# netease-youdao/EmotiVoice

Measured on NVIDIA H100. Metric: mel_frames_per_sec, higher is better.
Workload: dtype fp32 (fp32 storage + accumulate; tensor-core fp32 emulation: 3xTF32 prefix, bf16x3 after it)

## Files before the change

### emotivoice_b200/build.py

```python
import hashlib
import os
import subprocess
import sys

HERE = os.path.dirname(os.path.abspath(__file__))
CSRC = os.path.join(HERE, "csrc")
LIB_DIR = os.path.join(HERE, "lib")
LIB_PATH = os.path.join(LIB_DIR, "libemotivoice_b200.so")
INCLUDE = os.path.join(os.path.dirname(HERE), "include")

NVCC_FLAGS = ["-gencode", "arch=compute_90a,code=sm_90a", "-lineinfo", "-O3", "-std=c++17",
              "-Xcompiler", "-fPIC,-fvisibility=hidden", "-cudart", "static"]


def sources():
    return sorted(os.path.join(CSRC, f) for f in os.listdir(CSRC) if f.endswith(".cu"))


def _digest():
    h = hashlib.sha256()
    files = sources() + sorted(os.path.join(CSRC, f) for f in os.listdir(CSRC) if f.endswith(".cuh"))
    files.append(os.path.join(INCLUDE, "emotivoice_b200.h"))
    for f in files:
        h.update(os.path.basename(f).encode())
        with open(f, "rb") as fh:
            h.update(fh.read())
    h.update(" ".join(NVCC_FLAGS).encode())
    return h.hexdigest()


def nvcc_path():
    for c in (os.environ.get("NVCC"), "/usr/local/cuda/bin/nvcc", "nvcc"):
        if c and (os.path.isabs(c) and os.path.exists(c) or not os.path.isabs(c)):
            return c
    return "nvcc"


def build(force=False, verbose=True):
    import fcntl
    if not force and _up_to_date(_digest()):
        if verbose:
            print("emotivoice_b200.build: up to date, not recompiled", flush=True)
        return LIB_PATH
    os.makedirs(LIB_DIR, exist_ok=True)
    with open(os.path.join(LIB_DIR, ".build.lock"), "w") as lock:
        fcntl.flock(lock, fcntl.LOCK_EX)
        try:
            return _build_locked(force, verbose)
        finally:
            fcntl.flock(lock, fcntl.LOCK_UN)


def _up_to_date(dig):
    stamp = os.path.join(LIB_DIR, "build.stamp")
    if not (os.path.exists(LIB_PATH) and os.path.exists(stamp)):
        return False
    with open(stamp) as f:
        return f.read().strip() == dig


def _build_locked(force, verbose):
    stamp = os.path.join(LIB_DIR, "build.stamp")
    dig = _digest()
    if not force and _up_to_date(dig):
        if verbose:
            print("emotivoice_b200.build: up to date (sources digest %s), not recompiled" % dig[:12], flush=True)
        return LIB_PATH
    objs = []
    procs = []
    for src in sources():
        obj = os.path.join(LIB_DIR, os.path.basename(src)[:-3] + ".o")
        objs.append(obj)
        cmd = [nvcc_path()] + NVCC_FLAGS + ["-I", INCLUDE, "-c", src, "-o", obj]
        if verbose:
            print(" ".join(cmd), flush=True)
        procs.append((src, subprocess.Popen(cmd, stdout=subprocess.PIPE, stderr=subprocess.STDOUT)))
    serialised = []
    for src, p in procs:
        out, _ = p.communicate()
        if p.returncode != 0:
            sys.stderr.write(out.decode())
            raise RuntimeError("nvcc failed on %s" % src)
        if verbose and out.strip():
            print(out.decode())
        if b"C7520" in out:
            if not verbose:
                sys.stderr.write(out.decode())
            serialised.append(os.path.basename(src))
    if serialised:
        raise RuntimeError("ptxas serialised wgmma instructions (warning C7520, reason above) in %s; a wgmma on a path ptxas cannot "
                           "prove warp-uniform is one cause" % ", ".join(serialised))
    cmd = [nvcc_path(), "-shared", "-o", LIB_PATH] + objs + ["-cudart", "static",
                                                           "-gencode", "arch=compute_90a,code=sm_90a"]
    if verbose:
        print(" ".join(cmd), flush=True)
    subprocess.check_call(cmd)
    with open(stamp, "w") as f:
        f.write(dig)
    if verbose:
        print("emotivoice_b200.build: compiled %d sources with nvcc for sm_90a (digest %s)" % (len(objs), dig[:12]), flush=True)
    return LIB_PATH


if __name__ == "__main__":
    print(build(force="--force" in sys.argv))
```

### emotivoice_b200/csrc/conv1d_tc.cu

```cuda
#include <cstdio>
#include <cstdlib>

#include "ev_common.cuh"
#include "tc_common.cuh"

namespace ev {

namespace tc {

struct Plan {
  int BN, mt, kbg, planes;
  int rows_pad;
  int a_plane_bytes, b_plane_bytes, a_stage_bytes, b_stage_bytes;
  int a_stages, b_stages;
  int ngroups;
  int ksplit;
  int acc_cols;
  int tiles_m, tiles_n, total_tiles;
  int smem_total;
};

__host__ __device__ inline bool make_plan(const ConvParams& p, int mode, int BN, int mt, int kbg, int min_b_stages, Plan* o, int b_target = 4) {
  Plan q;
  q.planes = (mode == 1 || mode == 3) ? 2 : 1;
  const int cpg = mode >= 2 ? 8 : 4;
  q.kbg = kbg;
  q.mt = mt;
  q.BN = BN;
  if (mt * q.BN > 2 * ACC_REGS) return false;
  q.acc_cols = mt * q.BN;
  const int rows = BM * mt + (p.K - 1) * p.dil;
  q.rows_pad = ((rows + 7) / 8) * 8 + 8 / q.kbg;
  q.a_plane_bytes = q.kbg * q.rows_pad * 16;
  q.b_plane_bytes = q.kbg * q.BN * 16;
  q.a_stage_bytes = q.planes * q.a_plane_bytes;
  q.b_stage_bytes = q.planes * q.b_plane_bytes;
  const int budget = 227 * 1024 - 1024;
  const int n_cb = (p.Cin + cpg * q.kbg - 1) / (cpg * q.kbg);
  if (min_b_stages > n_cb * p.K) min_b_stages = n_cb * p.K;
  if (min_b_stages < 2) min_b_stages = 2;
  if (2 * q.a_stage_bytes + min_b_stages * q.b_stage_bytes > budget) return false;
  q.a_stages = 2;
  q.b_stages = 2;
  while (q.b_stages < MAX_B_STAGES && q.b_stages < n_cb * p.K &&
         q.a_stages * q.a_stage_bytes + (q.b_stages + 1) * q.b_stage_bytes <= budget && q.b_stages < b_target) ++q.b_stages;
  while (q.a_stages < MAX_A_STAGES && q.a_stages < n_cb &&
         (q.a_stages + 1) * q.a_stage_bytes + q.b_stages * q.b_stage_bytes <= budget && q.a_stages < 6) ++q.a_stages;
  while (q.b_stages < MAX_B_STAGES && q.b_stages < n_cb * p.K &&
         q.a_stages * q.a_stage_bytes + (q.b_stages + 1) * q.b_stage_bytes <= budget) ++q.b_stages;
  while (q.a_stages < MAX_A_STAGES && q.a_stages < n_cb &&
         (q.a_stages + 1) * q.a_stage_bytes + q.b_stages * q.b_stage_bytes <= budget) ++q.a_stages;
  q.ngroups = q.a_stages >= 6 ? 6 : (q.a_stages >= 3 ? 3 : (q.a_stages >= 2 ? 2 : 1));
  q.tiles_m = (p.L + BM * mt - 1) / (BM * mt);
  q.tiles_n = (p.Cout + q.BN - 1) / q.BN;
  q.ksplit = 1;
  q.total_tiles = p.B * q.tiles_m * q.tiles_n;
  q.smem_total = 1024 + q.a_stages * q.a_stage_bytes + q.b_stages * q.b_stage_bytes;
  *o = q;
  return true;
}

__device__ __forceinline__ void splitk_reduce_store(const ConvParams& p, int S, size_t per, size_t e, int b, int row, int col, int len) {
  float4 o = make_float4(0.f, 0.f, 0.f, 0.f);
  if (row < len) {
    for (int z = 0; z < S; ++z) {
      const float4 v = *reinterpret_cast<const float4*>(p.splitk_ws + (size_t)z * per + e);
      o.x += v.x; o.y += v.y; o.z += v.z; o.w += v.w;
    }
    if (p.bias) {
      const float4 b4 = __ldg(reinterpret_cast<const float4*>(p.bias + (size_t)b * p.bias_bs + col));
      o.x += b4.x; o.y += b4.y; o.z += b4.z; o.w += b4.w;
    }
    if (p.out_act != EV_ACT_NONE) {
      o.x = act_apply(o.x, p.out_act, 0.f); o.y = act_apply(o.y, p.out_act, 0.f);
      o.z = act_apply(o.z, p.out_act, 0.f); o.w = act_apply(o.w, p.out_act, 0.f);
    }
    if (p.res) {
      const float4 r4 = *reinterpret_cast<const float4*>(p.res + e);
      o.x += r4.x; o.y += r4.y; o.z += r4.z; o.w += r4.w;
    }
    if (p.acc != EV_ACC_STORE) {
      const float4 q4 = *reinterpret_cast<const float4*>(p.out + e);
      o.x += q4.x; o.y += q4.y; o.z += q4.z; o.w += q4.w;
      if (p.acc == EV_ACC_ADD_DIV) { o.x /= p.div; o.y /= p.div; o.z /= p.div; o.w /= p.div; }
    }
  }
  *reinterpret_cast<float4*>(p.out + e) = o;
}

template <int MODE, int MT, int KBG, int BN>
__global__ void __launch_bounds__(NTHREADS, 1) conv1d_tc_kernel(ConvParams p, Plan pl) {
  constexpr bool SPLIT3 = (MODE == 1);
  constexpr bool X3B = (MODE == 3);
  constexpr bool BF16 = (MODE == 2) || X3B;
  constexpr int PLANES = (SPLIT3 || X3B) ? 2 : 1;
  constexpr int CPG = BF16 ? 8 : 4;
  constexpr int KB = CPG * KBG;
  constexpr int NK8 = KBG / 2;
  constexpr int GSH = (KBG == 8 ? 3 : 2);
  constexpr int NA = BN / 2;
  constexpr int NCW = NCONS / 32;
  static_assert(BN % 16 == 0 && MT * BN <= 2 * ACC_REGS, "accumulators of the tile exceed the register budget");
  extern __shared__ __align__(128) uint8_t smem_raw[];
  const int tid = threadIdx.x;
  const int warp = __shfl_sync(0xffffffffu, tid >> 5, 0);
  const int lane = tid & 31;

  uint64_t* bars = reinterpret_cast<uint64_t*>(smem_raw);
  uint8_t* a_tiles = smem_raw + 1024;
  uint8_t* b_tiles = a_tiles + pl.a_stages * pl.a_stage_bytes;
  const uint32_t bar_base = smem_u32(bars);
  auto a_full = [&](int s) { return bar_base + 8u * s; };
  auto a_empty = [&](int s) { return bar_base + 8u * (MAX_A_STAGES + s); };
  auto b_full = [&](int s) { return bar_base + 8u * (2 * MAX_A_STAGES + s); };
  auto b_empty = [&](int s) { return bar_base + 8u * (2 * MAX_A_STAGES + MAX_B_STAGES + s); };

  if (tid == 0) {
    for (int s = 0; s < pl.a_stages; ++s) { mbar_init(a_full(s), (NPWARPS / pl.ngroups) * 32); mbar_init(a_empty(s), NCW); }
    for (int s = 0; s < pl.b_stages; ++s) { mbar_init(b_full(s), 1); mbar_init(b_empty(s), NCW); }
    asm volatile("fence.mbarrier_init.release.cluster;" ::: "memory");
  }
  __syncthreads();

  asm volatile("griddepcontrol.launch_dependents;" ::: "memory");

  const int n_cb = (p.Cin + KB - 1) / KB;
  const int halo = ((p.K - 1) / 2) * p.dil;
  const int rows_a = BM * MT + (p.K - 1) * p.dil;
  const int tiles_per_b = pl.tiles_m * pl.tiles_n;

  int z_cur = 0;
  auto decode = [&](int tile, int& b, int& t0, int& n0, int& nt, int& len) {
    z_cur = tile % pl.ksplit;
    tile /= pl.ksplit;
    b = tile / tiles_per_b;
    const int r = tile - b * tiles_per_b;
    const int tm = r / pl.tiles_n, tn = r - tm * pl.tiles_n;
    t0 = tm * (BM * MT);
    n0 = tn * BN;
    nt = min(BN, p.Cout - n0);
    len = p.lens ? min(p.L, p.lens[b] * p.lens_mul) : p.L;
  };

  if (warp < NCW) {
    asm volatile("griddepcontrol.wait;" ::: "memory");
    const int wg = warp >> 2, wl = warp & 3;
    const bool split = pl.ksplit > 1;
    const bool has_res = p.res != nullptr && !split;
    const int oact = split ? EV_ACT_NONE : p.out_act, accm = split ? EV_ACC_STORE : p.acc;
    const uint32_t a_lbo = (uint32_t)pl.rows_pad * 16u, b_lbo = (uint32_t)BN * 16u;
    const uint64_t a_desc0 = make_desc(0u, a_lbo, 128u), b_desc0 = make_desc(0u, b_lbo, 128u);
    const uint32_t a_tap = (uint32_t)p.dil * 16u, a_k8 = 2u * a_lbo;
    float acc[MT][NA];
#pragma unroll
    for (int mt = 0; mt < MT; ++mt)
#pragma unroll
      for (int i = 0; i < NA; ++i) acc[mt][i] = 0.f;
    auto release = [&](int sb, int sa) {
      __syncwarp();
      if (lane == 0) {
        mbar_arrive(b_empty(sb));
        if (sa >= 0) mbar_arrive(a_empty(sa));
      }
    };
    int a_cnt = 0, b_cnt = 0;
    for (int tile = blockIdx.x; tile < pl.total_tiles; tile += gridDim.x) {
      int b, t0, n0, nt, len;
      decode(tile, b, t0, n0, nt, len);
      float* ob = (split ? p.splitk_ws + (size_t)z_cur * p.B * p.L * p.Cout : p.out) + (size_t)b * p.L * p.Cout;
      const float* rb = has_res ? p.res + (size_t)b * p.L * p.Cout : nullptr;
      const bool active = t0 < len;
      if (active) {
        const int cb_lo = (z_cur * n_cb) / pl.ksplit, cb_hi = ((z_cur + 1) * n_cb) / pl.ksplit;
        int prev_sb = -1, prev_sa = -1;
        for (int cb = cb_lo; cb < cb_hi; ++cb, ++a_cnt) {
          const int sa = a_cnt % pl.a_stages;
          const int nk8 = min(KB, p.Cin - cb * KB) / (2 * CPG);
          mbar_wait(a_full(sa), (a_cnt / pl.a_stages) & 1);
          const uint64_t a_hi0 = desc_advance(a_desc0, smem_u32(a_tiles + sa * pl.a_stage_bytes) + (uint32_t)(wg * 64) * 16u);
          for (int j = 0; j < p.K; ++j, ++b_cnt) {
            const int sb = b_cnt % pl.b_stages;
            mbar_wait(b_full(sb), (b_cnt / pl.b_stages) & 1);
            const uint64_t b_hi0 = desc_advance(b_desc0, smem_u32(b_tiles + sb * pl.b_stage_bytes));
            const uint64_t a_j = desc_advance(a_hi0, (uint32_t)j * a_tap);
            if (nk8 == NK8) {
              tap_chain<MODE, BN, NK8>(acc, a_j, a_k8, (uint32_t)pl.a_plane_bytes, b_hi0, (uint32_t)pl.b_plane_bytes, (cb - cb_lo) | j);
              wgmma_wait<1>();
            } else {
              tap_chain_short<MODE, BN>(acc, a_j, a_k8, (uint32_t)pl.a_plane_bytes, b_hi0, (uint32_t)pl.b_plane_bytes, (cb - cb_lo) | j, nk8);
              wgmma_wait<1>();
            }
            if (prev_sb >= 0) release(prev_sb, prev_sa);
            prev_sb = sb;
            prev_sa = j == p.K - 1 ? sa : -1;
          }
        }
        wgmma_wait<0>();
        release(prev_sb, prev_sa);
      }
      const float* __restrict__ bias = (p.bias && !split) ? p.bias + (size_t)b * p.bias_bs + n0 : nullptr;
#pragma unroll
      for (int mt = 0; mt < MT; ++mt) {
#pragma unroll
        for (int i = 0; i < NA; i += 2) {
          const int c = frag_col(i, lane);
          const int row = t0 + mt * BM + wg * 64 + frag_row(i, lane, wl);
          if (c >= nt || row >= p.L) continue;
          const size_t off = (size_t)row * p.Cout + n0 + c;
          float2 o = make_float2(0.f, 0.f);
          if (active && row < len) {
            o = make_float2(acc[mt][i], acc[mt][i + 1]);
            if (bias) {
              const float2 b2 = __ldg(reinterpret_cast<const float2*>(bias + c));
              o.x += b2.x; o.y += b2.y;
            }
            if (oact != EV_ACT_NONE) { o.x = act_apply(o.x, oact, 0.f); o.y = act_apply(o.y, oact, 0.f); }
            if (has_res) {
              const float2 r2 = *reinterpret_cast<const float2*>(rb + off);
              o.x += r2.x; o.y += r2.y;
            }
            if (accm != EV_ACC_STORE) {
              const float2 q2 = *reinterpret_cast<const float2*>(ob + off);
              o.x += q2.x; o.y += q2.y;
              if (accm == EV_ACC_ADD_DIV) { o.x /= p.div; o.y /= p.div; }
            }
          }
          *reinterpret_cast<float2*>(ob + off) = o;
        }
      }
    }
  } else if (warp < W_WLOAD) {
    asm volatile("griddepcontrol.wait;" ::: "memory");
    const int pwarp = warp - NCW;
    const int wpg = NPWARPS / pl.ngroups;
    const int grp = pwarp / wpg;
    const int gt = (pwarp - grp * wpg) * 32 + lane;
    const int GT = wpg * 32;
    const bool lrelu = (p.in_act == EV_ACT_LRELU);
    const float slope = p.in_slope;
    const int total = rows_a * KBG;
    int a_cnt = 0;
    for (int tile = blockIdx.x; tile < pl.total_tiles; tile += gridDim.x) {
      int b, t0, n0, nt, len;
      decode(tile, b, t0, n0, nt, len);
      if (t0 >= len) continue;
      const float* __restrict__ xb = p.x + (size_t)b * p.L * p.Cin;
      const int cb_lo = (z_cur * n_cb) / pl.ksplit, cb_hi = ((z_cur + 1) * n_cb) / pl.ksplit;
      for (int cb = cb_lo; cb < cb_hi; ++cb, ++a_cnt) {
        if (a_cnt % pl.ngroups != grp) continue;
        const int s = a_cnt % pl.a_stages;
        const int c0 = cb * KB;
        const int ngran = min(KB, p.Cin - c0) / CPG;
        uint8_t* dst = a_tiles + s * pl.a_stage_bytes;
        constexpr int ALD = BF16 ? A_LD / 2 : A_LD;
        constexpr int NW = BF16 ? 2 : 1;
        for (int base = 0; base < total; base += GT * ALD) {
          float4 v[ALD * NW];
#pragma unroll
          for (int u = 0; u < ALD; ++u) {
            const int idx = base + u * GT + gt;
            const int r = idx >> GSH, g = idx & (KBG - 1);
            const int row = t0 - halo + r;
            const bool ok = idx < total && g < ngran && row >= 0 && row < len;
            const float* src = xb + (size_t)row * p.Cin + c0 + g * CPG;
#pragma unroll
            for (int w = 0; w < NW; ++w)
              v[u * NW + w] = ok ? __ldg(reinterpret_cast<const float4*>(src + 4 * w)) : make_float4(0.f, 0.f, 0.f, 0.f);
          }
          if (base == 0) mbar_wait(a_empty(s), ((a_cnt / pl.a_stages) & 1) ^ 1);
#pragma unroll
          for (int u = 0; u < ALD; ++u) {
            const int idx = base + u * GT + gt;
            const int r = idx >> GSH, g = idx & (KBG - 1);
            if (idx < total && g < ngran) {
#pragma unroll
              for (int w = 0; w < NW; ++w) {
                float4& t = v[u * NW + w];
                if (lrelu) {
                  t.x = t.x > 0.f ? t.x : t.x * slope;
                  t.y = t.y > 0.f ? t.y : t.y * slope;
                  t.z = t.z > 0.f ? t.z : t.z * slope;
                  t.w = t.w > 0.f ? t.w : t.w * slope;
                }
              }
              uint8_t* d = dst + ((size_t)g * pl.rows_pad + r) * 16;
              if (BF16) {
                const float4 t0 = v[u * NW], t1 = v[u * NW + NW - 1];
                uint4 q;
                q.x = pack_bf16(t0.x, t0.y); q.y = pack_bf16(t0.z, t0.w);
                q.z = pack_bf16(t1.x, t1.y); q.w = pack_bf16(t1.z, t1.w);
                *reinterpret_cast<uint4*>(d) = q;
                if (X3B) {
                  uint4 l;
                  l.x = pack_bf16(t0.x - __uint_as_float(q.x << 16), t0.y - __uint_as_float(q.x & 0xffff0000u));
                  l.y = pack_bf16(t0.z - __uint_as_float(q.y << 16), t0.w - __uint_as_float(q.y & 0xffff0000u));
                  l.z = pack_bf16(t1.x - __uint_as_float(q.z << 16), t1.y - __uint_as_float(q.z & 0xffff0000u));
                  l.w = pack_bf16(t1.z - __uint_as_float(q.w << 16), t1.w - __uint_as_float(q.w & 0xffff0000u));
                  *reinterpret_cast<uint4*>(d + pl.a_plane_bytes) = l;
                }
              } else {
                const float4 t = v[u * NW];
                const float4 h = make_float4(to_tf32(t.x), to_tf32(t.y), to_tf32(t.z), to_tf32(t.w));
                *reinterpret_cast<float4*>(d) = h;
                if (SPLIT3) {
                  const float4 l = make_float4(to_tf32(t.x - h.x), to_tf32(t.y - h.y), to_tf32(t.z - h.z), to_tf32(t.w - h.w));
                  *reinterpret_cast<float4*>(d + pl.a_plane_bytes) = l;
                }
              }
            }
          }
        }
        fence_proxy_async();
        mbar_arrive(a_full(s));
      }
    }
  } else {
    if (lane == 0) {
      asm volatile("griddepcontrol.wait;" ::: "memory");
      const int cin4 = p.Cin / CPG;
      const int bnp = p.Cout < 128 ? p.Cout : 128;
      const size_t plane = (size_t)p.K * cin4 * p.Cout * 4;
      const size_t tile_stride = (size_t)p.K * cin4 * bnp * 4;
      int b_cnt = 0;
      for (int tile = blockIdx.x; tile < pl.total_tiles; tile += gridDim.x) {
        int b, t0, n0, nt, len;
        decode(tile, b, t0, n0, nt, len);
        if (t0 >= len) continue;
        const float* wt = p.w + (size_t)(n0 / bnp) * tile_stride + (size_t)(n0 % bnp) * 4;
        const int cb_lo = (z_cur * n_cb) / pl.ksplit, cb_hi = ((z_cur + 1) * n_cb) / pl.ksplit;
        for (int cb = cb_lo; cb < cb_hi; ++cb) {
          const int ngran = min(KB, p.Cin - cb * KB) / CPG;
          for (int j = 0; j < p.K; ++j, ++b_cnt) {
            const int sb = b_cnt % pl.b_stages;
            mbar_wait(b_empty(sb), ((b_cnt / pl.b_stages) & 1) ^ 1);
            mbar_expect_tx(b_full(sb), (uint32_t)(PLANES * ngran * nt * 16));
            const uint32_t dst = smem_u32(b_tiles + sb * pl.b_stage_bytes);
            const float* src = wt + ((size_t)j * cin4 + (size_t)cb * KBG) * bnp * 4;
            if (nt == bnp) {
              bulk_g2s(dst, src, (uint32_t)(ngran * nt * 16), b_full(sb));
              if (PLANES == 2) bulk_g2s(dst + (uint32_t)pl.b_plane_bytes, src + plane, (uint32_t)(ngran * nt * 16), b_full(sb));
            } else {
              for (int g = 0; g < ngran; ++g) {
                bulk_g2s(dst + (uint32_t)(g * BN * 16), src + (size_t)g * bnp * 4, (uint32_t)(nt * 16), b_full(sb));
                if (PLANES == 2) bulk_g2s(dst + (uint32_t)(pl.b_plane_bytes + g * BN * 16), src + plane + (size_t)g * bnp * 4, (uint32_t)(nt * 16), b_full(sb));
              }
            }
          }
        }
      }
    }
    __syncwarp();
  }
}

__global__ void __launch_bounds__(256) splitk_reduce_kernel(ConvParams p, int S) {
  pdl_entry();
  const size_t per = (size_t)p.B * p.L * p.Cout;
  const size_t i4 = (size_t)blockIdx.x * blockDim.x + threadIdx.x;
  if (i4 * 4 >= per) return;
  const size_t e = i4 * 4;
  const int col = (int)(e % p.Cout);
  const size_t rowg = e / p.Cout;
  const int b = (int)(rowg / p.L), row = (int)(rowg % p.L);
  const int len = p.lens ? min(p.L, p.lens[b] * p.lens_mul) : p.L;
  splitk_reduce_store(p, S, per, e, b, row, col, len);
}

}

using TcKernel = void (*)(ConvParams, tc::Plan);
template <int MODE, int KBG>
static TcKernel tc_kernel_tile(int mt, int bn) {
  using namespace tc;
  switch (bn) {
    case 128: return mt == 1 ? conv1d_tc_kernel<MODE, 1, KBG, 128> : nullptr;
    case 112: return mt == 1 ? conv1d_tc_kernel<MODE, 1, KBG, 112> : nullptr;
    case 96: return mt == 1 ? conv1d_tc_kernel<MODE, 1, KBG, 96> : nullptr;
    case 80: return mt == 1 ? conv1d_tc_kernel<MODE, 1, KBG, 80> : nullptr;
    case 64: return mt == 2 ? conv1d_tc_kernel<MODE, 2, KBG, 64> : mt == 1 ? conv1d_tc_kernel<MODE, 1, KBG, 64> : nullptr;
    case 48: return mt == 2 ? conv1d_tc_kernel<MODE, 2, KBG, 48> : mt == 1 ? conv1d_tc_kernel<MODE, 1, KBG, 48> : nullptr;
    case 32: return mt == 4 ? conv1d_tc_kernel<MODE, 4, KBG, 32> : mt == 2 ? conv1d_tc_kernel<MODE, 2, KBG, 32>
                  : mt == 1 ? conv1d_tc_kernel<MODE, 1, KBG, 32> : nullptr;
    case 16: return mt == 4 ? conv1d_tc_kernel<MODE, 4, KBG, 16> : mt == 2 ? conv1d_tc_kernel<MODE, 2, KBG, 16>
                  : mt == 1 ? conv1d_tc_kernel<MODE, 1, KBG, 16> : nullptr;
    default: return nullptr;
  }
}
static TcKernel tc_kernel(int mode, int kbg, int mt, int bn) {
  if (mode == 1) return kbg == 4 ? tc_kernel_tile<1, 4>(mt, bn) : nullptr;
  if (mode == 3) return kbg == 8 ? tc_kernel_tile<3, 8>(mt, bn) : tc_kernel_tile<3, 4>(mt, bn);
  if (mode == 2) return kbg == 8 ? tc_kernel_tile<2, 8>(mt, bn) : tc_kernel_tile<2, 4>(mt, bn);
  return kbg == 8 ? tc_kernel_tile<0, 8>(mt, bn) : tc_kernel_tile<0, 4>(mt, bn);
}

void preload_conv1d_tc() {
  for (int mode = 0; mode < 4; ++mode)
    for (int kbg = 4; kbg <= 8; kbg += 4)
      for (int bn = 16; bn <= 128; bn += 16)
        for (int mt = 1; mt <= 4 && mt * bn <= 128; mt *= 2)
          if (const TcKernel k = tc_kernel(mode, kbg, mt, bn)) cudaFuncSetAttribute(k, cudaFuncAttributeMaxDynamicSharedMemorySize, 227 * 1024);
  cudaFuncAttributes fa;
  cudaFuncGetAttributes(&fa, tc::splitk_reduce_kernel);
  cudaGetLastError();
}

static int validate_conv1d_tc(const ConvParams& p, int mode) {
  EV_CHECK_ARG(p.B > 0 && p.L > 0, "conv1d_tc: bad problem B=%d L=%d", p.B, p.L);
  EV_CHECK_ARG(p.Cin % (mode >= 2 ? 16 : 8) == 0, "conv1d_tc: Cin=%d must be a multiple of %d", p.Cin, mode >= 2 ? 16 : 8);
  EV_CHECK_ARG(p.Cout % 16 == 0 && (p.Cout <= 128 || p.Cout % 128 == 0), "conv1d_tc: Cout=%d must be a multiple of 16, and of 128 above 128", p.Cout);
  EV_CHECK_ARG(p.K >= 1 && (p.K & 1) && p.dil >= 1, "conv1d_tc: K=%d must be odd, dil=%d >= 1", p.K, p.dil);
  EV_CHECK_ARG(p.in_act == EV_ACT_NONE || p.in_act == EV_ACT_LRELU, "conv1d_tc: unsupported input activation");
  return EV_OK;
}

int tc_shape_kbg(const ConvParams& p, int mode) {
  tc::Plan pl;
  const int bn_max = p.Cout <= 128 ? p.Cout : 128;
  return (mode != 1 && tc::make_plan(p, mode, bn_max, 1, 8, 4, &pl)) ? 8 : 4;
}

static int apply_ksplit(const ConvParams& p, int mode, tc::Plan* pl) {
  const size_t per = (size_t)p.B * p.L * p.Cout;
  if (p.ksplit > 1 && (p.splitk_ws || p.splitk_cap == (size_t)-1)) {
    int S = p.ksplit;
    const int cpg = mode >= 2 ? 8 : 4;
    const int n_cb = (p.Cin + cpg * pl->kbg - 1) / (cpg * pl->kbg);
    if (S > n_cb) S = n_cb;
    if ((size_t)S * per > p.splitk_cap) { set_error("conv1d_tc: split-K scratch too small (%zu < %zu floats)", p.splitk_cap, (size_t)S * per); return EV_EWORKSPACE; }
    if (S > 1) {
      pl->ksplit = S;
      pl->total_tiles *= S;
    }
  }
  return EV_OK;
}

static int plan_conv1d_tc(const ConvParams& p, int mode, tc::Plan* out) {
  EV_TRY(validate_conv1d_tc(p, mode));
  const int bn_thresh = 24, mt_thresh = 120;
  const long long tiles128 = (long long)((p.L + tc::BM - 1) / tc::BM) * p.B;
  int BN = p.Cout <= 128 ? p.Cout : 128;
  while (BN >= 64 && (BN / 2) % 16 == 0 && tiles128 * ((p.Cout + BN - 1) / BN) < bn_thresh) BN /= 2;
  int mt = tiles128 >= 4 * mt_thresh ? 4 : (tiles128 >= 2 * mt_thresh ? 2 : 1);
  tc::Plan pl;
  const int kbg = tc_shape_kbg(p, mode);
  for (;; mt >>= 1) {
    if (tc::make_plan(p, mode, BN, mt, kbg, 4, &pl)) break;
    if (tc::make_plan(p, mode, BN, mt, kbg, 2, &pl)) break;
    if (mt == 1) { set_error("conv1d_tc: tile does not fit in shared memory / accumulator registers (K=%d dil=%d Cout=%d)", p.K, p.dil, p.Cout); return EV_EINVAL; }
  }
  EV_TRY(apply_ksplit(p, mode, &pl));
  *out = pl;
  return EV_OK;
}

int debug_tc_plan(const ConvParams& p, int mode, int* v) {
  tc::Plan pl;
  const int rc = plan_conv1d_tc(p, mode, &pl);
  if (rc != EV_OK) return rc;
  v[0] = pl.BN; v[1] = pl.mt; v[2] = pl.kbg; v[3] = pl.a_stages; v[4] = pl.b_stages; v[5] = pl.ngroups;
  v[6] = pl.ksplit; v[7] = pl.acc_cols; v[8] = pl.smem_total; v[9] = pl.total_tiles; v[10] = pl.rows_pad;
  return EV_OK;
}

static int dispatch_tc(const ConvParams& p, int mode, const tc::Plan& pl, cudaStream_t st) {
  static std::atomic<uint64_t> attr_devs{0};
  if (first_use_on_device(attr_devs)) preload_conv1d_tc();
  const TcKernel k = tc_kernel(mode, pl.kbg, pl.mt, pl.BN);
  EV_CHECK_ARG(k, "conv1d_tc: no kernel for mode %d, KBG %d, MT %d, BN %d", mode, pl.kbg, pl.mt, pl.BN);
  const int grid = pl.total_tiles < sm_count() ? pl.total_tiles : sm_count();
  return launch("conv1d_tc_kernel", k, (unsigned)grid, tc::NTHREADS, pl.smem_total, st, p, pl);
}

int launch_conv1d_tc(const ConvParams& p, int mode, cudaStream_t st) {
  tc::Plan pl;
  EV_TRY(plan_conv1d_tc(p, mode, &pl));
  const size_t per = (size_t)p.B * p.L * p.Cout;
  const int rc = dispatch_tc(p, mode, pl, st);
  if (rc != EV_OK || pl.ksplit == 1) return rc;
  const size_t n4 = per / 4;
  return launch("splitk_reduce_kernel", tc::splitk_reduce_kernel, (unsigned)((n4 + 255) / 256), 256, 0, st, p, pl.ksplit);
}

}
```

Before: 126,500.

## Prefetch first weight stages before PDL grid-dependency wait in conv kernel

The weight-loader warp now issues bulk copies for the first block's initial B stages before griddepcontrol.wait, because the weights do not depend on the previous kernel. This overlaps weight fetch with the tail of the preceding launch. The consumer drains those early stages when the first tile is skipped. The change also adds an optional globaltimer timeline instrumentation build, compiled out by default.

```diff
diff --git a/emotivoice_b200/build.py b/emotivoice_b200/build.py
--- a/emotivoice_b200/build.py
+++ b/emotivoice_b200/build.py
@@ -66,12 +66,21 @@
         if verbose:
             print("emotivoice_b200.build: up to date (sources digest %s), not recompiled" % dig[:12], flush=True)
         return LIB_PATH
+    _compile(LIB_PATH, LIB_DIR, NVCC_FLAGS, verbose)
+    with open(stamp, "w") as f:
+        f.write(dig)
+    if verbose:
+        print("emotivoice_b200.build: compiled %d sources with nvcc for sm_90a (digest %s)" % (len(sources()), dig[:12]), flush=True)
+    return LIB_PATH
+
+
+def _compile(lib_path, obj_dir, flags, verbose):
     objs = []
     procs = []
     for src in sources():
-        obj = os.path.join(LIB_DIR, os.path.basename(src)[:-3] + ".o")
+        obj = os.path.join(obj_dir, os.path.basename(src)[:-3] + ".o")
         objs.append(obj)
-        cmd = [nvcc_path()] + NVCC_FLAGS + ["-I", INCLUDE, "-c", src, "-o", obj]
+        cmd = [nvcc_path()] + flags + ["-I", INCLUDE, "-c", src, "-o", obj]
         if verbose:
             print(" ".join(cmd), flush=True)
         procs.append((src, subprocess.Popen(cmd, stdout=subprocess.PIPE, stderr=subprocess.STDOUT)))
@@ -90,17 +99,22 @@
     if serialised:
         raise RuntimeError("ptxas serialised wgmma instructions (warning C7520, reason above) in %s; a wgmma on a path ptxas cannot "
                            "prove warp-uniform is one cause" % ", ".join(serialised))
-    cmd = [nvcc_path(), "-shared", "-o", LIB_PATH] + objs + ["-cudart", "static",
+    cmd = [nvcc_path(), "-shared", "-o", lib_path] + objs + ["-cudart", "static",
                                                            "-gencode", "arch=compute_90a,code=sm_90a"]
     if verbose:
         print(" ".join(cmd), flush=True)
     subprocess.check_call(cmd)
-    with open(stamp, "w") as f:
-        f.write(dig)
-    if verbose:
-        print("emotivoice_b200.build: compiled %d sources with nvcc for sm_90a (digest %s)" % (len(objs), dig[:12]), flush=True)
-    return LIB_PATH
+
+
+def build_timeline(out_dir, verbose=True):
+    os.makedirs(out_dir, exist_ok=True)
+    path = os.path.join(out_dir, "libemotivoice_b200_timeline.so")
+    _compile(path, out_dir, NVCC_FLAGS + ["-DEV_TC_TIMELINE"], verbose)
+    return path
 
 
 if __name__ == "__main__":
-    print(build(force="--force" in sys.argv))
+    if "--timeline" in sys.argv:
+        print(build_timeline(sys.argv[sys.argv.index("--timeline") + 1]))
+    else:
+        print(build(force="--force" in sys.argv))
diff --git a/emotivoice_b200/csrc/conv1d_tc.cu b/emotivoice_b200/csrc/conv1d_tc.cu
--- a/emotivoice_b200/csrc/conv1d_tc.cu
+++ b/emotivoice_b200/csrc/conv1d_tc.cu
@@ -7,6 +7,30 @@
 namespace ev {
 
 namespace tc {
+
+#ifdef EV_TC_TIMELINE
+constexpr int TL_SLOTS = 512, TL_N = 96;
+enum : int {
+  TL_CONS_ENTRY = 0, TL_CONS_WAITED, TL_MMA_FIRST, TL_MMA_LAST, TL_EPI_END, TL_PROD_ENTRY, TL_PROD_WAITED, TL_LOAD_ENTRY,
+  TL_LOAD_WAITED, TL_EPI_FIRST,
+  TL_A_START = 16,
+  TL_A_READY = TL_A_START + TL_N,
+  TL_B_ISSUE = TL_A_READY + TL_N,
+  TL_B_SEEN = TL_B_ISSUE + TL_N,
+  TL_A_SEEN = TL_B_SEEN + TL_N,
+};
+static_assert(TL_A_SEEN + TL_N <= TL_SLOTS, "timeline record overflows its slots");
+__device__ unsigned long long* g_tc_timeline = nullptr;
+__device__ __forceinline__ void tl_stamp(int slot, int i = 0) {
+  if (g_tc_timeline == nullptr || i >= TL_N) return;
+  unsigned long long t;
+  asm volatile("mov.u64 %0, %%globaltimer;" : "=l"(t) :: "memory");
+  g_tc_timeline[(size_t)blockIdx.x * TL_SLOTS + slot + i] = t;
+}
+#define EV_TL(...) tl_stamp(__VA_ARGS__)
+#else
+#define EV_TL(...) ((void)0)
+#endif
 
 struct Plan {
   int BN, mt, kbg, planes;
@@ -105,6 +129,11 @@
   const int tid = threadIdx.x;
   const int warp = __shfl_sync(0xffffffffu, tid >> 5, 0);
   const int lane = tid & 31;
+  if (lane == 0) {
+    if (warp == 0) EV_TL(TL_CONS_ENTRY);
+    if (warp == NCW) EV_TL(TL_PROD_ENTRY);
+    if (warp == W_WLOAD) EV_TL(TL_LOAD_ENTRY);
+  }
 
   uint64_t* bars = reinterpret_cast<uint64_t*>(smem_raw);
   uint8_t* a_tiles = smem_raw + 1024;
@@ -144,6 +173,7 @@
 
   if (warp < NCW) {
     asm volatile("griddepcontrol.wait;" ::: "memory");
+    if (tid == 0) EV_TL(TL_CONS_WAITED);
     const int wg = warp >> 2, wl = warp & 3;
     const bool split = pl.ksplit > 1;
     const bool has_res = p.res != nullptr && !split;
@@ -177,10 +207,15 @@
           const int sa = a_cnt % pl.a_stages;
           const int nk8 = min(KB, p.Cin - cb * KB) / (2 * CPG);
           mbar_wait(a_full(sa), (a_cnt / pl.a_stages) & 1);
+          if (tid == 0) EV_TL(TL_A_SEEN, a_cnt);
           const uint64_t a_hi0 = desc_advance(a_desc0, smem_u32(a_tiles + sa * pl.a_stage_bytes) + (uint32_t)(wg * 64) * 16u);
           for (int j = 0; j < p.K; ++j, ++b_cnt) {
             const int sb = b_cnt % pl.b_stages;
             mbar_wait(b_full(sb), (b_cnt / pl.b_stages) & 1);
+            if (tid == 0) {
+              EV_TL(TL_B_SEEN, b_cnt);
+              if (b_cnt == 0) EV_TL(TL_MMA_FIRST);
+            }
             const uint64_t b_hi0 = desc_advance(b_desc0, smem_u32(b_tiles + sb * pl.b_stage_bytes));
             const uint64_t a_j = desc_advance(a_hi0, (uint32_t)j * a_tap);
             if (nk8 == NK8) {
@@ -195,8 +230,17 @@
             prev_sa = j == p.K - 1 ? sa : -1;
           }
         }
+        if (tid == 0) EV_TL(TL_MMA_LAST);
         wgmma_wait<0>();
         release(prev_sb, prev_sa);
+      } else if (tile == (int)blockIdx.x) {
+        const int cb_lo = (z_cur * n_cb) / pl.ksplit, cb_hi = ((z_cur + 1) * n_cb) / pl.ksplit;
+        const int early = min(pl.b_stages, (cb_hi - cb_lo) * p.K);
+        for (int i = 0; i < early; ++i, ++b_cnt) {
+          const int sb = b_cnt % pl.b_stages;
+          mbar_wait(b_full(sb), (b_cnt / pl.b_stages) & 1);
+          release(sb, -1);
+        }
       }
       const float* __restrict__ bias = (p.bias && !split) ? p.bias + (size_t)b * p.bias_bs + n0 : nullptr;
 #pragma unroll
@@ -228,9 +272,14 @@
           *reinterpret_cast<float2*>(ob + off) = o;
         }
       }
+      if (tid == 0) {
+        if (tile == (int)blockIdx.x) EV_TL(TL_EPI_FIRST);
+        EV_TL(TL_EPI_END);
+      }
     }
   } else if (warp < W_WLOAD) {
     asm volatile("griddepcontrol.wait;" ::: "memory");
+    if (tid == NCONS) EV_TL(TL_PROD_WAITED);
     const int pwarp = warp - NCW;
     const int wpg = NPWARPS / pl.ngroups;
     const int grp = pwarp / wpg;
@@ -249,6 +298,7 @@
       for (int cb = cb_lo; cb < cb_hi; ++cb, ++a_cnt) {
         if (a_cnt % pl.ngroups != grp) continue;
         const int s = a_cnt % pl.a_stages;
+        if (gt == 0) EV_TL(TL_A_START, a_cnt);
         const int c0 = cb * KB;
         const int ngran = min(KB, p.Cin - c0) / CPG;
         uint8_t* dst = a_tiles + s * pl.a_stage_bytes;
@@ -312,41 +362,52 @@
         }
         fence_proxy_async();
         mbar_arrive(a_full(s));
+        if (gt == 0) EV_TL(TL_A_READY, a_cnt);
       }
     }
   } else {
     if (lane == 0) {
-      asm volatile("griddepcontrol.wait;" ::: "memory");
       const int cin4 = p.Cin / CPG;
       const int bnp = p.Cout < 128 ? p.Cout : 128;
       const size_t plane = (size_t)p.K * cin4 * p.Cout * 4;
       const size_t tile_stride = (size_t)p.K * cin4 * bnp * 4;
+      auto copy_stage = [&](int b_cnt, int n0, int nt, int cb, int j) {
+        const int ngran = min(KB, p.Cin - cb * KB) / CPG;
+        const int sb = b_cnt % pl.b_stages;
+        mbar_wait(b_empty(sb), ((b_cnt / pl.b_stages) & 1) ^ 1);
+        mbar_expect_tx(b_full(sb), (uint32_t)(PLANES * ngran * nt * 16));
+        EV_TL(TL_B_ISSUE, b_cnt);
+        const uint32_t dst = smem_u32(b_tiles + sb * pl.b_stage_bytes);
+        const float* src = p.w + (size_t)(n0 / bnp) * tile_stride + (size_t)(n0 % bnp) * 4 + ((size_t)j * cin4 + (size_t)cb * KBG) * bnp * 4;
+        if (nt == bnp) {
+          bulk_g2s(dst, src, (uint32_t)(ngran * nt * 16), b_full(sb));
+          if (PLANES == 2) bulk_g2s(dst + (uint32_t)pl.b_plane_bytes, src + plane, (uint32_t)(ngran * nt * 16), b_full(sb));
+        } else {
+          for (int g = 0; g < ngran; ++g) {
+            bulk_g2s(dst + (uint32_t)(g * BN * 16), src + (size_t)g * bnp * 4, (uint32_t)(nt * 16), b_full(sb));
+            if (PLANES == 2) bulk_g2s(dst + (uint32_t)(pl.b_plane_bytes + g * BN * 16), src + plane + (size_t)g * bnp * 4, (uint32_t)(nt * 16), b_full(sb));
+          }
+        }
+      };
+      const int z0 = (int)blockIdx.x % pl.ksplit;
+      const int n00 = (((int)blockIdx.x / pl.ksplit) % pl.tiles_n) * BN, nt0 = min(BN, p.Cout - n00);
+      const int cb_lo0 = (z0 * n_cb) / pl.ksplit, cb_hi0 = ((z0 + 1) * n_cb) / pl.ksplit;
+      const int early = min(pl.b_stages, (cb_hi0 - cb_lo0) * p.K);
+      for (int i = 0; i < early; ++i) copy_stage(i, n00, nt0, cb_lo0 + i / p.K, i % p.K);
+      asm volatile("griddepcontrol.wait;" ::: "memory");
+      EV_TL(TL_LOAD_WAITED);
       int b_cnt = 0;
       for (int tile = blockIdx.x; tile < pl.total_tiles; tile += gridDim.x) {
         int b, t0, n0, nt, len;
         decode(tile, b, t0, n0, nt, len);
-        if (t0 >= len) continue;
-        const float* wt = p.w + (size_t)(n0 / bnp) * tile_stride + (size_t)(n0 % bnp) * 4;
+        if (t0 >= len) {
+          if (tile == (int)blockIdx.x) b_cnt = early;
+          continue;
+        }
         const int cb_lo = (z_cur * n_cb) / pl.ksplit, cb_hi = ((z_cur + 1) * n_cb) / pl.ksplit;
-        for (int cb = cb_lo; cb < cb_hi; ++cb) {
-          const int ngran = min(KB, p.Cin - cb * KB) / CPG;
-          for (int j = 0; j < p.K; ++j, ++b_cnt) {
-            const int sb = b_cnt % pl.b_stages;
-            mbar_wait(b_empty(sb), ((b_cnt / pl.b_stages) & 1) ^ 1);
-            mbar_expect_tx(b_full(sb), (uint32_t)(PLANES * ngran * nt * 16));
-            const uint32_t dst = smem_u32(b_tiles + sb * pl.b_stage_bytes);
-            const float* src = wt + ((size_t)j * cin4 + (size_t)cb * KBG) * bnp * 4;
-            if (nt == bnp) {
-              bulk_g2s(dst, src, (uint32_t)(ngran * nt * 16), b_full(sb));
-              if (PLANES == 2) bulk_g2s(dst + (uint32_t)pl.b_plane_bytes, src + plane, (uint32_t)(ngran * nt * 16), b_full(sb));
-            } else {
-              for (int g = 0; g < ngran; ++g) {
-                bulk_g2s(dst + (uint32_t)(g * BN * 16), src + (size_t)g * bnp * 4, (uint32_t)(nt * 16), b_full(sb));
-                if (PLANES == 2) bulk_g2s(dst + (uint32_t)(pl.b_plane_bytes + g * BN * 16), src + plane + (size_t)g * bnp * 4, (uint32_t)(nt * 16), b_full(sb));
-              }
-            }
-          }
-        }
+        for (int cb = cb_lo; cb < cb_hi; ++cb)
+          for (int j = 0; j < p.K; ++j, ++b_cnt)
+            if (b_cnt >= early) copy_stage(b_cnt, n0, nt, cb, j);
       }
     }
     __syncwarp();
@@ -483,3 +544,9 @@
 }
 
 }
+
+#ifdef EV_TC_TIMELINE
+extern "C" EV_API int ev_debug_tc_timeline(unsigned long long* buf) {
+  return cudaMemcpyToSymbol(ev::tc::g_tc_timeline, &buf, sizeof(buf)) == cudaSuccess ? EV_OK : EV_ECUDA;
+}
+#endif
```

After: 126,000, median of 6. No clear change (-0.4%).
